# menyifang/MIMO

Measured on NVIDIA H100. Metric: frames/sec @ 512x512x24f, 20 DDIM steps, higher is better.
Workload: dtype fp16

## Files before the change

### mimo_b200/csrc/attn_spatial.cu

```cuda
#include <cuda_runtime.h>

#include "../../include/mimo_b200.h"
#include "attn_common.h"
#include "host_util.h"
#include "ptx.cuh"
#include "wgmma.cuh"

namespace mimo {

template <int DP>
struct AttnCfg {
  static constexpr int NCH = (DP + 63) / 64;
  static constexpr int NWG = DP >= 160 ? 1 : 2;
  static constexpr int QROWS = 64 * NWG;
  static constexpr int kThreads = 128 * NWG + 32;
  static constexpr int kQChunk = QROWS * 128;
  static constexpr int kQBytes = NCH * kQChunk;
  static constexpr int kKVStageBytes = 2 * NCH * kChunkBytes;
  static constexpr int kFit = (227 * 1024 - 1024 - 256 - kQBytes) / kKVStageBytes;
  static constexpr int KVST = kFit < 3 ? kFit : 3;
  static constexpr int kSmemBytes = kQBytes + KVST * kKVStageBytes + 1024 + 256;
  static_assert(KVST >= 1, "K/V tile does not fit");
};

template <int DP, bool kBf16>
__global__ void __launch_bounds__(AttnCfg<DP>::kThreads, 1)
attn_spatial_kernel(const __grid_constant__ CUtensorMap tmQ, const __grid_constant__ CUtensorMap tmK,
                    const __grid_constant__ CUtensorMap tmV, const __grid_constant__ CUtensorMap tmBK,
                    const __grid_constant__ CUtensorMap tmBV, AttnArgs a) {
  using Cfg = AttnCfg<DP>;
  using C = Cvt<kBf16>;
  constexpr int NCH = Cfg::NCH, KVST = Cfg::KVST, kProd = 4 * Cfg::NWG;
  extern __shared__ uint8_t smem_raw[];
  uint8_t* smem = reinterpret_cast<uint8_t*>((reinterpret_cast<uintptr_t>(smem_raw) + 1023) & ~uintptr_t(1023));
  uint8_t* sQ = smem;
  uint8_t* sKV = sQ + Cfg::kQBytes;
  uint64_t* bars = reinterpret_cast<uint64_t*>(sKV + KVST * Cfg::kKVStageBytes);
  uint64_t* q_full = bars;
  uint64_t* kv_full = bars + 1;
  uint64_t* kv_empty = kv_full + KVST;

  const int warp = __shfl_sync(0xffffffffu, threadIdx.x >> 5, 0);
  const int lane = threadIdx.x & 31;
  const int q_tile = blockIdx.x;
  const int h = blockIdx.y;
  const int n = blockIdx.z;
  pdl_launch_dependents();
  pdl_wait();
  const int bidx = __shfl_sync(0xffffffffu, a.bank_index ? a.bank_index[n] : -1, 0);
  const int T = a.n_self_tiles + (bidx >= 0 ? a.n_bank_tiles : 0);

  if (warp == kProd && lane == 0) {
    tma_prefetch_desc(&tmQ);
    tma_prefetch_desc(&tmK);
    tma_prefetch_desc(&tmV);
    if (bidx >= 0) {
      tma_prefetch_desc(&tmBK);
      tma_prefetch_desc(&tmBV);
    }
  }
  if (warp == kProd && lane == 1) {
    mbar_init(q_full, 1);
    for (int s = 0; s < KVST; ++s) {
      mbar_init(&kv_full[s], 1);
      mbar_init(&kv_empty[s], kProd);
    }
    fence_mbar_init();
  }
  __syncthreads();

  if (warp == kProd && lane == 0) {
    mbar_expect_tx(q_full, Cfg::kQBytes);
#pragma unroll
    for (int ch = 0; ch < NCH; ++ch) tma_load_4d(sQ + ch * Cfg::kQChunk, &tmQ, q_full, ch * 64, h, q_tile * Cfg::QROWS, n);
    for (int j = 0; j < T; ++j) {
      const int stage = j % KVST;
      const uint32_t phase = (j / KVST) & 1u;
      mbar_wait(&kv_empty[stage], phase ^ 1u);
      uint8_t* sk = sKV + stage * Cfg::kKVStageBytes;
      uint8_t* sv = sk + NCH * kChunkBytes;
      mbar_expect_tx(&kv_full[stage], Cfg::kKVStageBytes);
      const bool bank = j >= a.n_self_tiles;
      const int row0 = (bank ? j - a.n_self_tiles : j) * BKV;
      const int img = bank ? bidx : n;
      const CUtensorMap* mk = bank ? &tmBK : &tmK;
      const CUtensorMap* mv = bank ? &tmBV : &tmV;
#pragma unroll
      for (int ch = 0; ch < NCH; ++ch) {
        tma_load_4d(sk + ch * kChunkBytes, mk, &kv_full[stage], ch * 64, h, row0, img);
        tma_load_4d(sv + ch * kChunkBytes, mv, &kv_full[stage], ch * 64, h, row0, img);
      }
    }
  } else if (warp < kProd) {
    const int wg = warp >> 2;
    const int rbase = wg * 64 + (warp & 3) * 16 + (lane >> 2);
    const int q2 = (lane & 3) * 2;
    const uint32_t q_addr = smem_u32(sQ) + wg * (64 * 128);
    float o[DP / 2];
    float m[2] = {-INFINITY, -INFINITY}, l[2] = {0.f, 0.f};
    mbar_wait(q_full, 0);
    for (int j = 0; j < T; ++j) {
      const int stage = j % KVST;
      const bool bank = j >= a.n_self_tiles;
      const int len = bank ? a.lb : a.lq;
      const int row0 = (bank ? j - a.n_self_tiles : j) * BKV;
      int valid = len - row0;
      if (valid > BKV) valid = BKV;
      mbar_wait(&kv_full[stage], (j / KVST) & 1u);
      const uint32_t k_addr = smem_u32(sKV + stage * Cfg::kKVStageBytes);
      const uint32_t v_addr = k_addr + NCH * kChunkBytes;

      float s[BKV / 2];
      wgmma_fence();
#pragma unroll
      for (int ks = 0; ks < DP / 16; ++ks) {
        const uint32_t off = (ks & 3) * 32;
        Wgmma<BKV, kBf16>::ss(s, make_smem_desc_sw128(q_addr + (ks >> 2) * Cfg::kQChunk + off, 16, 1024),
                              make_smem_desc_sw128(k_addr + (ks >> 2) * kChunkBytes + off, 16, 1024), ks != 0 ? 1u : 0u);
      }
      wgmma_commit();
      wgmma_wait<0>();
      reg_fence(s);

      float mx[2] = {-INFINITY, -INFINITY};
#pragma unroll
      for (int jn = 0; jn < BKV / 8; ++jn)
#pragma unroll
        for (int e = 0; e < 4; ++e) {
          if (8 * jn + q2 + (e & 1) < valid)
            mx[e >> 1] = fmaxf(mx[e >> 1], s[4 * jn + e]);
          else
            s[4 * jn + e] = -INFINITY;
        }
      float alpha[2], m_new[2];
#pragma unroll
      for (int r = 0; r < 2; ++r) {
        mx[r] = fmaxf(mx[r], __shfl_xor_sync(0xffffffffu, mx[r], 1));
        mx[r] = fmaxf(mx[r], __shfl_xor_sync(0xffffffffu, mx[r], 2));
        m_new[r] = fmaxf(m[r], mx[r] * a.scale_log2);
        alpha[r] = exp2f(m[r] - m_new[r]);
      }
      uint32_t pa[BKV / 16][4];
      float rowsum[2] = {0.f, 0.f};
#pragma unroll
      for (int kk = 0; kk < BKV / 16; ++kk)
#pragma unroll
        for (int i = 0; i < 4; ++i) {
          const int e = 8 * kk + 2 * i;
          const int r = i & 1;
          const float p0 = exp2f(fmaf(s[e], a.scale_log2, -m_new[r]));
          const float p1 = exp2f(fmaf(s[e + 1], a.scale_log2, -m_new[r]));
          rowsum[r] += p0 + p1;
          pa[kk][i] = C::pack(p0, p1);
        }
#pragma unroll
      for (int r = 0; r < 2; ++r) {
        l[r] = l[r] * alpha[r] + rowsum[r];
        m[r] = m_new[r];
      }
      if (j > 0) {
#pragma unroll
        for (int i = 0; i < DP / 2; ++i) o[i] *= alpha[(i >> 1) & 1];
      }
      wgmma_fence();
#pragma unroll
      for (int kk = 0; kk < BKV / 16; ++kk) {
        Wgmma<DP, kBf16>::rs(o, pa[kk], make_smem_desc_sw128(v_addr + kk * 2048, kChunkBytes, 1024),
                             (j | kk) != 0 ? 1u : 0u);
      }
      wgmma_commit();
      wgmma_wait<0>();
      reg_fence(o);
      if (lane == 0) mbar_arrive(&kv_empty[stage]);
    }
#pragma unroll
    for (int r = 0; r < 2; ++r) {
      l[r] += __shfl_xor_sync(0xffffffffu, l[r], 1);
      l[r] += __shfl_xor_sync(0xffffffffu, l[r], 2);
      const float inv_l = 1.0f / l[r];
      const int qrow = q_tile * Cfg::QROWS + rbase + 8 * r;
      if (qrow < a.lq) {
        typename C::T* orow =
            static_cast<typename C::T*>(a.out) + (static_cast<long long>(n) * a.lq + qrow) * a.ld_out + h * a.d;
#pragma unroll
        for (int jn = 0; jn < DP / 8; ++jn)
          if (8 * jn + q2 < a.d)
            *reinterpret_cast<uint32_t*>(orow + 8 * jn + q2) = C::pack(o[4 * jn + 2 * r] * inv_l, o[4 * jn + 2 * r + 1] * inv_l);
      }
    }
  }
}

static int attn_tmap(CUtensorMap* m, int dtype, const void* base, int d, int heads, int len, int nimg, long long ld,
                     uint32_t rows = BKV);

template <int DP, bool kBf16>
static int launch_attn(const mimo_attn_params* p, const CUtensorMap& k, const CUtensorMap& v, const CUtensorMap& bk,
                       const CUtensorMap& bv, const AttnArgs& a, cudaStream_t st) {
  using Cfg = AttnCfg<DP>;
  auto kern = attn_spatial_kernel<DP, kBf16>;
  static bool attr_done = false;
  if (!attr_done) {
    cudaError_t e = cudaFuncSetAttribute(kern, cudaFuncAttributeMaxDynamicSharedMemorySize, Cfg::kSmemBytes);
    if (e != cudaSuccess) return set_cuda_error("cudaFuncSetAttribute(attn)", e);
    attr_done = true;
  }
  CUtensorMap q;
  if (int rc = attn_tmap(&q, p->dtype, p->q, p->d, p->heads, p->lq, p->n, p->ld_qkv, Cfg::QROWS)) return rc;
  const dim3 grid((p->lq + Cfg::QROWS - 1) / Cfg::QROWS, p->heads, p->n);
  cudaError_t e = launch_k(kern, grid, dim3(Cfg::kThreads), Cfg::kSmemBytes, st, q, k, v, bk, bv, a);
  if (e == cudaSuccess) e = cudaGetLastError();
  if (e != cudaSuccess) return set_cuda_error("attn launch", e);
  return MIMO_OK;
}

static int attn_tmap(CUtensorMap* m, int dtype, const void* base, int d, int heads, int len, int nimg, long long ld,
                     uint32_t rows) {
  const uint64_t dims[4] = {static_cast<uint64_t>(d), static_cast<uint64_t>(heads), static_cast<uint64_t>(len),
                            static_cast<uint64_t>(nimg)};
  const uint64_t str[3] = {static_cast<uint64_t>(d) * 2, static_cast<uint64_t>(ld) * 2,
                           static_cast<uint64_t>(len) * ld * 2};
  const uint32_t box[4] = {64, 1, rows, 1};
  return encode_tmap(m, dtype, 4, base, dims, str, box);
}

}

using namespace mimo;

extern "C" int mimo_attn_spatial(const mimo_attn_params* p, void* stream) {
  if (!p || !p->q || !p->k || !p->v || !p->out) return set_error(MIMO_ERR_ARG, "mimo_attn_spatial: null pointer");
  if (p->n <= 0 || p->lq <= 0 || p->heads <= 0 || p->d <= 0 || (p->d % 8) || p->d > 192 || (p->ld_qkv % 8) ||
      (p->ld_out % 8))
    return set_error(MIMO_ERR_ARG, "mimo_attn_spatial: need d % 8 == 0, d <= 192, leading dims % 8 == 0");
  const bool has_bank = p->bank_index && p->bank_k && p->bank_v && p->lb > 0;
  if (has_bank && (p->ld_bank % 8)) return set_error(MIMO_ERR_ARG, "mimo_attn_spatial: ld_bank % 8 != 0");
  if (int rc = ensure_device()) return rc;

  AttnArgs a;
  a.lq = p->lq;
  a.lb = has_bank ? p->lb : 0;
  a.heads = p->heads;
  a.d = p->d;
  a.dp = (p->d + 15) / 16 * 16;
  a.n_self_tiles = (p->lq + BKV - 1) / BKV;
  a.n_bank_tiles = has_bank ? (p->lb + BKV - 1) / BKV : 0;
  a.scale_log2 = p->scale * 1.4426950408889634f;
  a.bank_index = has_bank ? p->bank_index : nullptr;
  a.out = p->out;
  a.ld_out = p->ld_out;

  CUtensorMap tk, tv, tbk, tbv;
  if (int rc = attn_tmap(&tk, p->dtype, p->k, p->d, p->heads, p->lq, p->n, p->ld_qkv)) return rc;
  if (int rc = attn_tmap(&tv, p->dtype, p->v, p->d, p->heads, p->lq, p->n, p->ld_qkv)) return rc;
  if (has_bank) {
    const int nb = p->nb > 0 ? p->nb : 1;
    if (int rc = attn_tmap(&tbk, p->dtype, p->bank_k, p->d, p->heads, p->lb, nb, p->ld_bank)) return rc;
    if (int rc = attn_tmap(&tbv, p->dtype, p->bank_v, p->d, p->heads, p->lb, nb, p->ld_bank)) return rc;
  } else {
    tbk = tk;
    tbv = tv;
  }
  cudaStream_t st = static_cast<cudaStream_t>(stream);
  switch (a.dp) {
#define MIMO_ATTN_DP(DP) \
  case DP:               \
    return p->dtype == MIMO_BF16 ? launch_attn<DP, true>(p, tk, tv, tbk, tbv, a, st) \
                                 : launch_attn<DP, false>(p, tk, tv, tbk, tbv, a, st);
    MIMO_ATTN_DP(16) MIMO_ATTN_DP(32) MIMO_ATTN_DP(48) MIMO_ATTN_DP(64) MIMO_ATTN_DP(80) MIMO_ATTN_DP(96)
    MIMO_ATTN_DP(112) MIMO_ATTN_DP(128) MIMO_ATTN_DP(144) MIMO_ATTN_DP(160) MIMO_ATTN_DP(176) MIMO_ATTN_DP(192)
#undef MIMO_ATTN_DP
  }
  return set_error(MIMO_ERR_ARG, "mimo_attn_spatial: unsupported head dim");
}
```

### mimo_b200/csrc/ptx.cuh

```cuda
#pragma once
#include <cuda_fp16.h>
#include <cuda_bf16.h>
#include <cuda.h>
#include <stdint.h>
#include <stdio.h>

namespace mimo {

__device__ __forceinline__ uint32_t smem_u32(const void* p) {
  return static_cast<uint32_t>(__cvta_generic_to_shared(p));
}
__device__ __forceinline__ uint32_t lane_id() { return threadIdx.x & 31u; }

__device__ __forceinline__ bool elect_one() {
  uint32_t pred = 0;
  asm volatile(
      "{\n\t.reg .pred P;\n\telect.sync _|P, 0xffffffff;\n\tselp.u32 %0, 1, 0, P;\n\t}\n"
      : "=r"(pred));
  return pred != 0;
}

__device__ __forceinline__ void pdl_launch_dependents() { asm volatile("griddepcontrol.launch_dependents;" ::: "memory"); }
__device__ __forceinline__ void pdl_wait() { asm volatile("griddepcontrol.wait;" ::: "memory"); }

__device__ __forceinline__ void mbar_init(uint64_t* bar, uint32_t count) {
  asm volatile("mbarrier.init.shared::cta.b64 [%0], %1;" ::"r"(smem_u32(bar)), "r"(count));
}
__device__ __forceinline__ void fence_mbar_init() {
  asm volatile("fence.mbarrier_init.release.cluster;" ::: "memory");
}
__device__ __forceinline__ void mbar_expect_tx(uint64_t* bar, uint32_t bytes) {
  asm volatile("mbarrier.arrive.expect_tx.shared::cta.b64 _, [%0], %1;" ::"r"(smem_u32(bar)),
               "r"(bytes)
               : "memory");
}
__device__ __forceinline__ void mbar_arrive(uint64_t* bar) {
  asm volatile("mbarrier.arrive.shared::cta.b64 _, [%0];" ::"r"(smem_u32(bar)) : "memory");
}
__device__ __forceinline__ bool mbar_try_wait(uint64_t* bar, uint32_t parity) {
  uint32_t ok;
  asm volatile(
      "{\n\t.reg .pred p;\n\t"
      "mbarrier.try_wait.parity.shared::cta.b64 p, [%1], %2;\n\t"
      "selp.u32 %0, 1, 0, p;\n\t}\n"
      : "=r"(ok)
      : "r"(smem_u32(bar)), "r"(parity)
      : "memory");
  return ok != 0;
}
__device__ __forceinline__ bool mbar_test(uint64_t* bar, uint32_t parity) {
  uint32_t ok;
  asm volatile(
      "{\n\t.reg .pred p;\n\t"
      "mbarrier.test_wait.parity.shared::cta.b64 p, [%1], %2;\n\t"
      "selp.u32 %0, 1, 0, p;\n\t}\n"
      : "=r"(ok)
      : "r"(smem_u32(bar)), "r"(parity)
      : "memory");
  return ok != 0;
}
__device__ __forceinline__ void mbar_wait(uint64_t* bar, uint32_t parity) {
  uint32_t spins = 0;
  while (!mbar_try_wait(bar, parity)) {
    if (++spins > (1u << 26)) __trap();
  }
}

__device__ __forceinline__ void fence_proxy_async_smem() {
  asm volatile("fence.proxy.async.shared::cta;" ::: "memory");
}

__device__ __forceinline__ void tma_prefetch_desc(const CUtensorMap* m) {
  asm volatile("prefetch.tensormap [%0];" ::"l"(reinterpret_cast<uint64_t>(m)) : "memory");
}
__device__ __forceinline__ void tma_load_2d(void* smem_dst, const CUtensorMap* m, uint64_t* bar,
                                            int32_t c0, int32_t c1) {
  asm volatile(
      "cp.async.bulk.tensor.2d.shared::cluster.global.mbarrier::complete_tx::bytes"
      " [%0], [%1, {%3, %4}], [%2];"
      ::"r"(smem_u32(smem_dst)), "l"(reinterpret_cast<uint64_t>(m)), "r"(smem_u32(bar)), "r"(c0),
      "r"(c1)
      : "memory");
}
__device__ __forceinline__ void tma_load_3d(void* smem_dst, const CUtensorMap* m, uint64_t* bar,
                                            int32_t c0, int32_t c1, int32_t c2) {
  asm volatile(
      "cp.async.bulk.tensor.3d.shared::cluster.global.mbarrier::complete_tx::bytes"
      " [%0], [%1, {%3, %4, %5}], [%2];"
      ::"r"(smem_u32(smem_dst)), "l"(reinterpret_cast<uint64_t>(m)), "r"(smem_u32(bar)), "r"(c0),
      "r"(c1), "r"(c2)
      : "memory");
}
__device__ __forceinline__ void tma_load_4d(void* smem_dst, const CUtensorMap* m, uint64_t* bar,
                                            int32_t c0, int32_t c1, int32_t c2, int32_t c3) {
  asm volatile(
      "cp.async.bulk.tensor.4d.shared::cluster.global.mbarrier::complete_tx::bytes"
      " [%0], [%1, {%3, %4, %5, %6}], [%2];"
      ::"r"(smem_u32(smem_dst)), "l"(reinterpret_cast<uint64_t>(m)), "r"(smem_u32(bar)), "r"(c0),
      "r"(c1), "r"(c2), "r"(c3)
      : "memory");
}

__device__ __forceinline__ void tma_store_2d(const CUtensorMap* m, const void* smem_src, int32_t c0, int32_t c1) {
  asm volatile("cp.async.bulk.tensor.2d.global.shared::cta.bulk_group [%0, {%2, %3}], [%1];"
               ::"l"(reinterpret_cast<uint64_t>(m)), "r"(smem_u32(smem_src)), "r"(c0), "r"(c1)
               : "memory");
}
__device__ __forceinline__ void tma_store_4d(const CUtensorMap* m, const void* smem_src, int32_t c0, int32_t c1,
                                             int32_t c2, int32_t c3) {
  asm volatile("cp.async.bulk.tensor.4d.global.shared::cta.bulk_group [%0, {%2, %3, %4, %5}], [%1];"
               ::"l"(reinterpret_cast<uint64_t>(m)), "r"(smem_u32(smem_src)), "r"(c0), "r"(c1), "r"(c2), "r"(c3)
               : "memory");
}
__device__ __forceinline__ void tma_store_commit() { asm volatile("cp.async.bulk.commit_group;" ::: "memory"); }
__device__ __forceinline__ void tma_store_wait_read0() { asm volatile("cp.async.bulk.wait_group.read 0;" ::: "memory"); }
__device__ __forceinline__ void tma_store_wait_all() { asm volatile("cp.async.bulk.wait_group 0;" ::: "memory"); }

__device__ __forceinline__ void wgmma_fence() { asm volatile("wgmma.fence.sync.aligned;" ::: "memory"); }
__device__ __forceinline__ void wgmma_commit() { asm volatile("wgmma.commit_group.sync.aligned;" ::: "memory"); }
template <int N>
__device__ __forceinline__ void wgmma_wait() {
  asm volatile("wgmma.wait_group.sync.aligned %0;" ::"n"(N) : "memory");
}
template <int N>
__device__ __forceinline__ void reg_fence(float (&d)[N]) {
#pragma unroll
  for (int i = 0; i < N; ++i) asm volatile("" : "+f"(d[i])::"memory");
}

__device__ __forceinline__ uint64_t make_smem_desc_sw128(uint32_t smem_addr, uint32_t lbo_bytes,
                                                         uint32_t sbo_bytes) {
  uint64_t d = 0;
  d |= static_cast<uint64_t>((smem_addr & 0x3FFFFu) >> 4);
  d |= static_cast<uint64_t>((lbo_bytes >> 4) & 0x3FFFu) << 16;
  d |= static_cast<uint64_t>((sbo_bytes >> 4) & 0x3FFFu) << 32;
  d |= static_cast<uint64_t>(1) << 62;
  return d;
}

__device__ __forceinline__ float silu_f(float x) { return __fdividef(x, 1.0f + __expf(-x)); }
__device__ __forceinline__ float gelu_erf_f(float x) {
  return 0.5f * x * (1.0f + erff(x * 0.70710678118654752440f));
}

__device__ __forceinline__ float gelu_erf_fast(float x) {
  const float z = fabsf(x) * 0.70710678118654752440f;
  float t;
  asm("rcp.approx.ftz.f32 %0, %1;" : "=f"(t) : "f"(fmaf(0.3275911f, z, 1.0f)));
  float poly = fmaf(1.061405429f, t, -1.453152027f);
  poly = fmaf(poly, t, 1.421413741f);
  poly = fmaf(poly, t, -0.284496736f);
  poly = fmaf(poly, t, 0.254829592f);
  poly *= t;
  float e;
  asm("ex2.approx.ftz.f32 %0, %1;" : "=f"(e) : "f"(-z * z * 1.4426950408889634f));
  const float erf_abs = fmaf(-poly, e, 1.0f);
  const float erf_v = copysignf(erf_abs, x);
  return 0.5f * x * (1.0f + erf_v);
}

template <bool kBf16>
struct Cvt;
template <>
struct Cvt<false> {
  using T = __half;
  using T2 = __half2;
  static __device__ __forceinline__ float to_f(T v) { return __half2float(v); }
  static __device__ __forceinline__ T from_f(float v) { return __float2half_rn(v); }
  static __device__ __forceinline__ uint32_t pack(float a, float b) {
    __half2 h = __floats2half2_rn(a, b);
    return *reinterpret_cast<uint32_t*>(&h);
  }
  static __device__ __forceinline__ float2 unpack(uint32_t u) {
    return __half22float2(*reinterpret_cast<__half2*>(&u));
  }
};
template <>
struct Cvt<true> {
  using T = __nv_bfloat16;
  using T2 = __nv_bfloat162;
  static __device__ __forceinline__ float to_f(T v) { return __bfloat162float(v); }
  static __device__ __forceinline__ T from_f(float v) { return __float2bfloat16_rn(v); }
  static __device__ __forceinline__ uint32_t pack(float a, float b) {
    __nv_bfloat162 h = __floats2bfloat162_rn(a, b);
    return *reinterpret_cast<uint32_t*>(&h);
  }
  static __device__ __forceinline__ float2 unpack(uint32_t u) {
    return __bfloat1622float2(*reinterpret_cast<__nv_bfloat162*>(&u));
  }
};

}
```

Baseline: 5.733.

## Ping-pong warpgroups and overlap next QK^T with current PV in spatial attention

```diff
diff --git a/mimo_b200/csrc/attn_spatial.cu b/mimo_b200/csrc/attn_spatial.cu
--- a/mimo_b200/csrc/attn_spatial.cu
+++ b/mimo_b200/csrc/attn_spatial.cu
@@ -18,10 +18,60 @@
   static constexpr int kQBytes = NCH * kQChunk;
   static constexpr int kKVStageBytes = 2 * NCH * kChunkBytes;
   static constexpr int kFit = (227 * 1024 - 1024 - 256 - kQBytes) / kKVStageBytes;
-  static constexpr int KVST = kFit < 3 ? kFit : 3;
+  static constexpr int KVST = kFit < 4 ? kFit : 4;
+  static constexpr bool kLook = NWG == 2 && KVST >= 2 && DP <= 80;
   static constexpr int kSmemBytes = kQBytes + KVST * kKVStageBytes + 1024 + 256;
   static_assert(KVST >= 1, "K/V tile does not fit");
 };
+
+template <bool kMask, bool kBf16>
+__device__ __forceinline__ void softmax_tile(float (&s)[BKV / 2], int valid, int q2, float scale_log2, float (&m)[2],
+                                             float (&l)[2], float (&alpha)[2], uint32_t (&pa)[BKV / 16][4]) {
+  float mx[2] = {-INFINITY, -INFINITY};
+#pragma unroll
+  for (int jn = 0; jn < BKV / 8; ++jn)
+#pragma unroll
+    for (int e = 0; e < 4; ++e) {
+      if (!kMask || 8 * jn + q2 + (e & 1) < valid)
+        mx[e >> 1] = fmaxf(mx[e >> 1], s[4 * jn + e]);
+      else
+        s[4 * jn + e] = -INFINITY;
+    }
+  float m_new[2];
+#pragma unroll
+  for (int r = 0; r < 2; ++r) {
+    mx[r] = fmaxf(mx[r], __shfl_xor_sync(0xffffffffu, mx[r], 1));
+    mx[r] = fmaxf(mx[r], __shfl_xor_sync(0xffffffffu, mx[r], 2));
+    m_new[r] = fmaxf(m[r], mx[r] * scale_log2);
+    alpha[r] = ex2_ftz(m[r] - m_new[r]);
+  }
+  float rowsum[2] = {0.f, 0.f};
+#pragma unroll
+  for (int kk = 0; kk < BKV / 16; ++kk)
+#pragma unroll
+    for (int i = 0; i < 4; ++i) {
+      const int e = 8 * kk + 2 * i;
+      const int r = i & 1;
+      const float p0 = ex2_ftz(fmaf(s[e], scale_log2, -m_new[r]));
+      const float p1 = ex2_ftz(fmaf(s[e + 1], scale_log2, -m_new[r]));
+      rowsum[r] += p0 + p1;
+      pa[kk][i] = Cvt<kBf16>::pack(p0, p1);
+    }
+#pragma unroll
+  for (int r = 0; r < 2; ++r) {
+    l[r] = l[r] * alpha[r] + rowsum[r];
+    m[r] = m_new[r];
+  }
+}
+
+template <bool kBf16>
+__device__ __forceinline__ void softmax_step(float (&s)[BKV / 2], int valid, int q2, float scale_log2, float (&m)[2],
+                                             float (&l)[2], float (&alpha)[2], uint32_t (&pa)[BKV / 16][4]) {
+  if (valid < BKV)
+    softmax_tile<true, kBf16>(s, valid, q2, scale_log2, m, l, alpha, pa);
+  else
+    softmax_tile<false, kBf16>(s, valid, q2, scale_log2, m, l, alpha, pa);
+}
 
 template <int DP, bool kBf16>
 __global__ void __launch_bounds__(AttnCfg<DP>::kThreads, 1)
@@ -69,7 +119,8 @@
   }
   __syncthreads();
 
-  if (warp == kProd && lane == 0) {
+  if (warp == kProd) {
+    if (lane != 0) return;
     mbar_expect_tx(q_full, Cfg::kQBytes);
 #pragma unroll
     for (int ch = 0; ch < NCH; ++ch) tma_load_4d(sQ + ch * Cfg::kQChunk, &tmQ, q_full, ch * 64, h, q_tile * Cfg::QROWS, n);
@@ -91,102 +142,121 @@
         tma_load_4d(sv + ch * kChunkBytes, mv, &kv_full[stage], ch * 64, h, row0, img);
       }
     }
-  } else if (warp < kProd) {
-    const int wg = warp >> 2;
-    const int rbase = wg * 64 + (warp & 3) * 16 + (lane >> 2);
-    const int q2 = (lane & 3) * 2;
-    const uint32_t q_addr = smem_u32(sQ) + wg * (64 * 128);
-    float o[DP / 2];
-    float m[2] = {-INFINITY, -INFINITY}, l[2] = {0.f, 0.f};
-    mbar_wait(q_full, 0);
+    return;
+  }
+  const int wg = warp >> 2;
+  const int rbase = wg * 64 + (warp & 3) * 16 + (lane >> 2);
+  const int q2 = (lane & 3) * 2;
+  const uint32_t q_addr = smem_u32(sQ) + wg * (64 * 128);
+  const float scale_log2 = a.scale_log2;
+  auto tile_valid = [&](int j) {
+    const bool bank = j >= a.n_self_tiles;
+    const int valid = (bank ? a.lb : a.lq) - (bank ? j - a.n_self_tiles : j) * BKV;
+    return valid < BKV ? valid : BKV;
+  };
+  auto kv_addr = [&](int j) { return smem_u32(sKV + (j % KVST) * Cfg::kKVStageBytes); };
+  auto wait_kv = [&](int j) { mbar_wait(&kv_full[j % KVST], (j / KVST) & 1u); };
+  auto issue_s = [&](float (&s)[BKV / 2], uint32_t k_addr) {
+#pragma unroll
+    for (int ks = 0; ks < DP / 16; ++ks) {
+      const uint32_t off = (ks & 3) * 32;
+      Wgmma<BKV, kBf16>::ss(s, make_smem_desc_sw128(q_addr + (ks >> 2) * Cfg::kQChunk + off, 16, 1024),
+                            make_smem_desc_sw128(k_addr + (ks >> 2) * kChunkBytes + off, 16, 1024), ks != 0 ? 1u : 0u);
+    }
+  };
+  float o[DP / 2];
+  auto issue_pv = [&](const uint32_t (&pa)[BKV / 16][4], uint32_t v_addr, bool first) {
+#pragma unroll
+    for (int kk = 0; kk < BKV / 16; ++kk) {
+      Wgmma<DP, kBf16>::rs(o, pa[kk], make_smem_desc_sw128(v_addr + kk * 2048, kChunkBytes, 1024),
+                           (!first || kk != 0) ? 1u : 0u);
+    }
+  };
+  auto release = [&](int j) {
+    if (lane == 0) mbar_arrive(&kv_empty[j % KVST]);
+  };
+  float m[2] = {-INFINITY, -INFINITY}, l[2] = {0.f, 0.f}, alpha[2];
+  float s[BKV / 2];
+  uint32_t pa[BKV / 16][4];
+  mbar_wait(q_full, 0);
+
+  if constexpr (Cfg::kLook) {
+    const int bar_mine = 1 + wg, bar_other = 2 - wg;
+    if (wg == 1) bar_arrive(bar_other, 256);
+    wait_kv(0);
+    bar_sync(bar_mine, 256);
+    wgmma_fence();
+    issue_s(s, kv_addr(0));
+    wgmma_commit();
+    bar_arrive(bar_other, 256);
+    wgmma_wait<0>();
+    reg_fence(s);
+    softmax_step<kBf16>(s, tile_valid(0), q2, scale_log2, m, l, alpha, pa);
+    for (int j = 0; j + 1 < T; ++j) {
+      wait_kv(j + 1);
+      bar_sync(bar_mine, 256);
+      wgmma_fence();
+      issue_s(s, kv_addr(j + 1));
+      wgmma_commit();
+      issue_pv(pa, kv_addr(j) + NCH * kChunkBytes, j == 0);
+      wgmma_commit();
+      bar_arrive(bar_other, 256);
+      uint32_t pn[BKV / 16][4];
+      wgmma_wait<1>();
+      reg_fence(s);
+      softmax_step<kBf16>(s, tile_valid(j + 1), q2, scale_log2, m, l, alpha, pn);
+      wgmma_wait<0>();
+      reg_fence(o);
+      release(j);
+#pragma unroll
+      for (int i = 0; i < DP / 2; ++i) o[i] *= alpha[(i >> 1) & 1];
+#pragma unroll
+      for (int kk = 0; kk < BKV / 16; ++kk)
+#pragma unroll
+        for (int i = 0; i < 4; ++i) pa[kk][i] = __byte_perm(pa[kk][i], pn[kk][i], 0x7654);
+    }
+    bar_sync(bar_mine, 256);
+    wgmma_fence();
+    issue_pv(pa, kv_addr(T - 1) + NCH * kChunkBytes, T == 1);
+    wgmma_commit();
+    if (wg == 0) bar_arrive(bar_other, 256);
+    wgmma_wait<0>();
+    reg_fence(o);
+    release(T - 1);
+  } else {
     for (int j = 0; j < T; ++j) {
-      const int stage = j % KVST;
-      const bool bank = j >= a.n_self_tiles;
-      const int len = bank ? a.lb : a.lq;
-      const int row0 = (bank ? j - a.n_self_tiles : j) * BKV;
-      int valid = len - row0;
-      if (valid > BKV) valid = BKV;
-      mbar_wait(&kv_full[stage], (j / KVST) & 1u);
-      const uint32_t k_addr = smem_u32(sKV + stage * Cfg::kKVStageBytes);
-      const uint32_t v_addr = k_addr + NCH * kChunkBytes;
-
-      float s[BKV / 2];
+      wait_kv(j);
       wgmma_fence();
-#pragma unroll
-      for (int ks = 0; ks < DP / 16; ++ks) {
-        const uint32_t off = (ks & 3) * 32;
-        Wgmma<BKV, kBf16>::ss(s, make_smem_desc_sw128(q_addr + (ks >> 2) * Cfg::kQChunk + off, 16, 1024),
-                              make_smem_desc_sw128(k_addr + (ks >> 2) * kChunkBytes + off, 16, 1024), ks != 0 ? 1u : 0u);
-      }
+      issue_s(s, kv_addr(j));
       wgmma_commit();
       wgmma_wait<0>();
       reg_fence(s);
-
-      float mx[2] = {-INFINITY, -INFINITY};
-#pragma unroll
-      for (int jn = 0; jn < BKV / 8; ++jn)
-#pragma unroll
-        for (int e = 0; e < 4; ++e) {
-          if (8 * jn + q2 + (e & 1) < valid)
-            mx[e >> 1] = fmaxf(mx[e >> 1], s[4 * jn + e]);
-          else
-            s[4 * jn + e] = -INFINITY;
-        }
-      float alpha[2], m_new[2];
-#pragma unroll
-      for (int r = 0; r < 2; ++r) {
-        mx[r] = fmaxf(mx[r], __shfl_xor_sync(0xffffffffu, mx[r], 1));
-        mx[r] = fmaxf(mx[r], __shfl_xor_sync(0xffffffffu, mx[r], 2));
-        m_new[r] = fmaxf(m[r], mx[r] * a.scale_log2);
-        alpha[r] = exp2f(m[r] - m_new[r]);
-      }
-      uint32_t pa[BKV / 16][4];
-      float rowsum[2] = {0.f, 0.f};
-#pragma unroll
-      for (int kk = 0; kk < BKV / 16; ++kk)
-#pragma unroll
-        for (int i = 0; i < 4; ++i) {
-          const int e = 8 * kk + 2 * i;
-          const int r = i & 1;
-          const float p0 = exp2f(fmaf(s[e], a.scale_log2, -m_new[r]));
-          const float p1 = exp2f(fmaf(s[e + 1], a.scale_log2, -m_new[r]));
-          rowsum[r] += p0 + p1;
-          pa[kk][i] = C::pack(p0, p1);
-        }
-#pragma unroll
-      for (int r = 0; r < 2; ++r) {
-        l[r] = l[r] * alpha[r] + rowsum[r];
-        m[r] = m_new[r];
-      }
+      softmax_step<kBf16>(s, tile_valid(j), q2, scale_log2, m, l, alpha, pa);
       if (j > 0) {
 #pragma unroll
         for (int i = 0; i < DP / 2; ++i) o[i] *= alpha[(i >> 1) & 1];
       }
       wgmma_fence();
-#pragma unroll
-      for (int kk = 0; kk < BKV / 16; ++kk) {
-        Wgmma<DP, kBf16>::rs(o, pa[kk], make_smem_desc_sw128(v_addr + kk * 2048, kChunkBytes, 1024),
-                             (j | kk) != 0 ? 1u : 0u);
-      }
+      issue_pv(pa, kv_addr(j) + NCH * kChunkBytes, j == 0);
       wgmma_commit();
       wgmma_wait<0>();
       reg_fence(o);
-      if (lane == 0) mbar_arrive(&kv_empty[stage]);
-    }
-#pragma unroll
-    for (int r = 0; r < 2; ++r) {
-      l[r] += __shfl_xor_sync(0xffffffffu, l[r], 1);
-      l[r] += __shfl_xor_sync(0xffffffffu, l[r], 2);
-      const float inv_l = 1.0f / l[r];
-      const int qrow = q_tile * Cfg::QROWS + rbase + 8 * r;
-      if (qrow < a.lq) {
-        typename C::T* orow =
-            static_cast<typename C::T*>(a.out) + (static_cast<long long>(n) * a.lq + qrow) * a.ld_out + h * a.d;
-#pragma unroll
-        for (int jn = 0; jn < DP / 8; ++jn)
-          if (8 * jn + q2 < a.d)
-            *reinterpret_cast<uint32_t*>(orow + 8 * jn + q2) = C::pack(o[4 * jn + 2 * r] * inv_l, o[4 * jn + 2 * r + 1] * inv_l);
-      }
+      release(j);
+    }
+  }
+#pragma unroll
+  for (int r = 0; r < 2; ++r) {
+    l[r] += __shfl_xor_sync(0xffffffffu, l[r], 1);
+    l[r] += __shfl_xor_sync(0xffffffffu, l[r], 2);
+    const float inv_l = 1.0f / l[r];
+    const int qrow = q_tile * Cfg::QROWS + rbase + 8 * r;
+    if (qrow < a.lq) {
+      typename C::T* orow =
+          static_cast<typename C::T*>(a.out) + (static_cast<long long>(n) * a.lq + qrow) * a.ld_out + h * a.d;
+#pragma unroll
+      for (int jn = 0; jn < DP / 8; ++jn)
+        if (8 * jn + q2 < a.d)
+          *reinterpret_cast<uint32_t*>(orow + 8 * jn + q2) = C::pack(o[4 * jn + 2 * r] * inv_l, o[4 * jn + 2 * r + 1] * inv_l);
     }
   }
 }
diff --git a/mimo_b200/csrc/ptx.cuh b/mimo_b200/csrc/ptx.cuh
--- a/mimo_b200/csrc/ptx.cuh
+++ b/mimo_b200/csrc/ptx.cuh
@@ -126,6 +126,13 @@
 __device__ __forceinline__ void reg_fence(float (&d)[N]) {
 #pragma unroll
   for (int i = 0; i < N; ++i) asm volatile("" : "+f"(d[i])::"memory");
+}
+
+__device__ __forceinline__ void bar_sync(int id, int count) {
+  asm volatile("bar.sync %0, %1;" ::"r"(id), "r"(count) : "memory");
+}
+__device__ __forceinline__ void bar_arrive(int id, int count) {
+  asm volatile("bar.arrive %0, %1;" ::"r"(id), "r"(count) : "memory");
 }
 
 __device__ __forceinline__ uint64_t make_smem_desc_sw128(uint32_t smem_addr, uint32_t lbo_bytes,
@@ -138,6 +145,11 @@
   return d;
 }
 
+__device__ __forceinline__ float ex2_ftz(float x) {
+  float y;
+  asm("ex2.approx.ftz.f32 %0, %1;" : "=f"(y) : "f"(x));
+  return y;
+}
 __device__ __forceinline__ float silu_f(float x) { return __fdividef(x, 1.0f + __expf(-x)); }
 __device__ __forceinline__ float gelu_erf_f(float x) {
   return 0.5f * x * (1.0f + erff(x * 0.70710678118654752440f));
```

Result: faster. 6.191 (median of 6 runs) (+8.0%).
